# afiaka87/clip-guided-diffusion

Hardware: AMD Instinct MI355X
Metric: diffusion steps/sec (UNet+CLIP+grad) at 256x256 cutn=16 (higher is better)
Workload: dtype bf16x3 (split-bf16 MFMA, fp32 accumulate, fp32 storage); 1 GPU; BASELINE configs[1]: 256x256 class-cond UNet (554M), respace 250, cutn 16, batch 1/GPU, CLIP ViT-B/32, cgs 1000 tv 150 range 50, randomize_class, p_sample; global_batch=1, world_size_checked=1, collectives=none (single process)

## Files before the change

### clip-guided-diffusion_amd/csrc/capi.hip

```cpp
#include "../../include/cgd_mi355x.h"
#include "common.h"
#include "guidance.h"
#include "kernels.h"
#include "mfma_stage.h"
#include "net.h"

#define S(stream) ((hipStream_t)(stream))

extern "C" {

const char* cgd_version(void) { return "cgd_mi355x 0.1 (gfx950)"; }

int cgd_ctx_create(cgd_ctx** out, int device) {
  if (!out) return -3;
  cgd_ctx* ctx = new cgd_ctx();
  ctx->device = device;
  int prev = -1;
  (void)hipGetDevice(&prev);
  if (hipSetDevice(device) != hipSuccess) {
    delete ctx;
    return -1;
  }
  struct Restore {
    int d;
// ... 609 lines not shown
  return cgd_launch_conv_in(ctx, x, w, bias, y, Bn, H, W, Cin, Cout, S(stream));
}
int cgd_op_sr_stem(cgd_ctx* ctx, const float* x, const float* low, int B_low, int h, int w, const float* wpacked, const float* bias, float* y,
                   int ldy, int B, int H, int W, int Cout, void* stream) {
  CGD_NEED_CTX(ctx);
  return cgd_launch_sr_stem(ctx, x, low, B_low, h, w, wpacked, bias, y, ldy, B, H, W, Cout, S(stream));
}
int cgd_op_conv_thin_out(cgd_ctx* ctx, const float* x, int ldx, const float* w, const float* bias, float* y, int Bn, int H, int W,
                         int Cin, int Cout, void* stream) {
  CGD_NEED_CTX(ctx);
  return cgd_launch_conv_thin_out(ctx, x, ldx, w, bias, y, Bn, H, W, Cin, Cout, S(stream));
}
int64_t cgd_op_gn_scratch_floats(int B, int HW, int C) { return (int64_t)cgd_gn_scratch_floats(B, HW, C); }
int cgd_op_gn_fwd(cgd_ctx* ctx, const float* x, int ldx, float* y, int ldy, int B, int HW, int C, const float* gamma, const float* beta,
                  const float* film, int act, float eps, float* scratch, void* stream) {
  CGD_NEED_CTX(ctx);
  return cgd_launch_gn_fwd(ctx, x, ldx, y, ldy, B, HW, C, gamma, beta, film, 2 * C, act, eps, scratch, S(stream));
}
int cgd_op_gn_bwd(cgd_ctx* ctx, const float* x, int ldx, const float* dz, int lddz, float* dx, int lddx, const float* add, int ldadd,
                  int B, int HW, int C, int act, float* scratch, void* stream) {
  CGD_NEED_CTX(ctx);
  return cgd_launch_gn_bwd(ctx, x, ldx, dz, lddz, dx, lddx, add, ldadd, B, HW, C, act, scratch, S(stream));
}
int cgd_op_ln_fwd(cgd_ctx* ctx, const float* x, float* y, int rows, int C, const float* gamma, const float* beta, float eps, float* stats,
                  void* stream) {
  CGD_NEED_CTX(ctx);
  return cgd_launch_ln_fwd(ctx, x, C, y, C, rows, C, gamma, beta, eps, stats, S(stream));
}
int cgd_op_ln_bwd(cgd_ctx* ctx, const float* x, const float* dy, float* dx, int rows, int C, const float* gamma, const float* stats,
                  void* stream) {
  CGD_NEED_CTX(ctx);
  return cgd_launch_ln_bwd(ctx, x, C, dy, C, dx, C, nullptr, 0, rows, C, gamma, stats, S(stream));
}
int cgd_op_pool2x2(cgd_ctx* ctx, const float* in, float* out, int B, int Ho, int Wo, int C, float scale, void* stream) {
  CGD_NEED_CTX(ctx);
  return cgd_launch_pool2x2(ctx, in, C, out, C, nullptr, 0, B, Ho, Wo, C, scale, S(stream));
}
int cgd_op_upsample2x(cgd_ctx* ctx, const float* in, float* out, int B, int Ho, int Wo, int C, float scale, void* stream) {
  CGD_NEED_CTX(ctx);
  return cgd_launch_upsample2x(ctx, in, C, out, C, nullptr, 0, B, Ho, Wo, C, scale, S(stream));
}
int cgd_op_act(cgd_ctx* ctx, const float* x, const float* dy, float* out, int64_t n, int act, void* stream) {
  CGD_NEED_CTX(ctx);
  if (dy) return cgd_launch_act_bwd(ctx, x, dy, out, n, act, S(stream));
  return cgd_launch_act_fwd(ctx, x, out, n, act, S(stream));
}
// ... 41 lines not shown
```

### clip-guided-diffusion_amd/csrc/common.h

```cpp
#pragma once
#include <hip/hip_runtime.h>
#include <stdint.h>
#include <stdio.h>
#include <atomic>
#include <string>
#include <utility>
#include <vector>

inline std::atomic<unsigned long long> g_cgd_launches{0}, g_cgd_reduces{0};
#define CGD_LAUNCH(...)                                          \
  do {                                                           \
    g_cgd_launches.fetch_add(1, std::memory_order_relaxed);      \
    hipLaunchKernelGGL(__VA_ARGS__);                             \
  } while (0)

enum { CGD_PREC_F32 = 0, CGD_PREC_BF16X3 = 1, CGD_PREC_BF16 = 2 };

enum { CGD_PROF_GEMM = 0, CGD_PROF_HCONV = 1, CGD_PROF_GN = 2, CGD_PROF_WCONV = 3, CGD_PROF_KCONV = 4, CGD_PROF_WCONV_GNB = 5, CGD_PROF_KINDS = 6 };

struct ProfRec {
  hipEvent_t a = nullptr, b = nullptr;
  double flops = 0.0;
  int kind = 0;
  bool live = false;
};

struct SplitSrc {
  const float* ws = nullptr;
  const float* bias = nullptr;
  const float* R = nullptr;
  long stride = 0;
  int n = 0;
  int N = 0, ldr = 0;
  float alpha = 1.f;
};
struct PendingReduce {
  bool valid = false;
  SplitSrc src;
  float* C = nullptr;
  int ldc = 0, M = 0;
  hipStream_t stream = nullptr;
};

struct ChanStatsEntry {
  const float* C = nullptr;
  int ldc = 0, N = 0;
  long M = 0;
  float* buf = nullptr;
  size_t cap = 0;
  hipStream_t stream = nullptr;
  unsigned long long serial = 0;
  int kind = 0;
  int cnt = 128;
};
struct ChanSrc {
  const float* p0 = nullptr;
  const float* p1 = nullptr;
// ... 34 lines not shown
  int attn_x3 = 1;
  int attn_flash = 3;
  int fuse_act = 1;
  int fuse_gn_skip_m = 0;
  int fuse_gn_max_m = 1 << 30, fuse_gn_min_m = 4096;
  int fuse_gn = 1;
  int tile_order = 0;
  int hgemm_epi = 1;
  int hgemm_kg = 1;
  int weight_nt = 0;
  int kgemm_var = 0;
  int kgemm_big_m = 0, kgemm_big_n = 0;
  int kgemm_mode = 2, kgemm_max_m = 256;
  int hgemm_tm96 = 1;
  int hgemm_var = 1;
  int hgemm_mode = 1, hgemm_min_m = 64, hgemm_min_chunks = 4;
  PendingReduce pending;
  int defer_mode = 2;
  std::vector<ChanStatsEntry> chanstats;
  std::vector<float*> chanstats_retired;
  unsigned long long stats_serial = 1;
  unsigned long long device_allocs = 0;
  unsigned long long gn_record_merges = 0;
  bool last_wconv_bstat = false;
  int gn_epi = 3;
  std::vector<std::pair<const float*, int>> attn_fwd_path;
  std::vector<FragEntry> frag_cache;
  void* frag_tmp = nullptr;
  size_t frag_tmp_bytes = 0;
  bool prof_on = false;
  std::vector<ProfRec> prof_recs;
  std::vector<hipEvent_t> prof_pool;
  double prof_ms[CGD_PROF_KINDS] = {}, prof_flops[CGD_PROF_KINDS] = {}, prof_n[CGD_PROF_KINDS] = {};
};

struct ExactScope {
  cgd_ctx* ctx;
  int saved;
  explicit ExactScope(cgd_ctx* c) : ctx(c), saved(c->precision) { c->precision = CGD_PREC_F32; }
  ~ExactScope() { ctx->precision = saved; }
};

struct DeviceScope {
  int prev = -1;
  bool switched = false;
  explicit DeviceScope(const cgd_ctx* c) {
// ... 144 lines not shown
```

### clip-guided-diffusion_amd/csrc/kernels.h

```cpp
#pragma once
#include "common.h"

size_t cgd_gn_scratch_floats(int B, int HW, int C);
int cgd_launch_gn_fwd(cgd_ctx* ctx, const float* x, int ldx, float* y, int ldy, int B, int HW, int C, const float* gamma,
                      const float* beta, const float* film, int ldfilm, int act, float eps, float* scratch, hipStream_t s);
const float* cgd_gn_ab(const float* scratch, int B, int HW, int C);
const float* cgd_gn_coef(const float* scratch, int B, int HW, int C);
size_t cgd_gn_stats_offset(int B, int HW, int C);
int cgd_launch_gn_bwd(cgd_ctx* ctx, const float* x, int ldx, const float* dz, int lddz, float* dx, int lddx, const float* add,
                      int ldadd, int B, int HW, int C, int act, float* scratch, hipStream_t s, const float* add2 = nullptr,
                      int ldadd2 = 0);
int cgd_launch_gn_bwd_skip_gemm(cgd_ctx* ctx, GemmParams sk, const float* x, int ldx, const float* dz, int lddz, const float* add2, int ldadd2,
                                int B, int HW, int C, float* scratch, hipStream_t s, bool* done);
int cgd_launch_ln_fwd(cgd_ctx* ctx, const float* x, int ldx, float* y, int ldy, int rows, int C, const float* gamma,
                      const float* beta, float eps, float* stats, hipStream_t s);
int cgd_launch_ln_bwd(cgd_ctx* ctx, const float* x, int ldx, const float* dy, int lddy, float* dx, int lddx, const float* add,
                      int ldadd, int rows, int C, const float* gamma, const float* stats, hipStream_t s);

int cgd_launch_pool2x2(cgd_ctx* ctx, const float* in, int ldi, float* out, int ldo, const float* add, int ldadd, int B, int Ho,
                       int Wo, int C, float scale, hipStream_t s);
int cgd_launch_resample2x_pair(cgd_ctx* ctx, int up, const float* in0, int ldi0, float* out0, int ldo0, const float* in1, int ldi1, float* out1,
                               int ldo1, int B, int Ho, int Wo, int C, float scale, hipStream_t s);
int cgd_launch_upsample2x(cgd_ctx* ctx, const float* in, int ldi, float* out, int ldo, const float* add, int ldadd, int B, int Ho,
                          int Wo, int C, float scale, hipStream_t s);
int cgd_launch_copy2d(cgd_ctx* ctx, const float* a, int lda, const float* b, int ldb, float* out, int ldo, long rows, int C,
                      hipStream_t s);
int cgd_launch_concat2(cgd_ctx* ctx, const float* a, int lda, int Ca, const float* b, int ldb, int Cb, float* out, int ldo, long rows,
                       hipStream_t s);
int cgd_launch_act_fwd(cgd_ctx* ctx, const float* x, float* y, long n, int act, hipStream_t s);
int cgd_launch_act_bwd(cgd_ctx* ctx, const float* x, const float* dy, float* dx, long n, int act, hipStream_t s);
int cgd_launch_transpose(cgd_ctx* ctx, const float* in, int ldi, long si, float* out, int ldo, long so, int R, int Cc, int nb,
                         hipStream_t s);
int cgd_launch_timestep_embedding(cgd_ctx* ctx, const float* t, const float* freqs, float* out, int B, int dim, hipStream_t s);
int cgd_launch_embedding_add(cgd_ctx* ctx, const float* table, const int64_t* idx, float* out, int B, int dim, hipStream_t s);
// ... 112 lines not shown
```

### clip-guided-diffusion_amd/csrc/norm.hip

```cpp
#include "common.h"
#include "mfma_stage.h"
#include "kernels.h"

namespace {

constexpr int MAXJ = 4;
constexpr int GN_U = 4;

struct ColMap {
  int cq, TQ, rows, r, q0;
  bool active;
};
__device__ __forceinline__ ColMap col_map(int C) {
  ColMap m;
  m.cq = C >> 2;
  m.TQ = m.cq < 256 ? m.cq : 256;
  m.rows = 256 / m.TQ;
  m.r = threadIdx.x / m.TQ;
  m.q0 = threadIdx.x % m.TQ;
  m.active = m.r < m.rows;
  return m;
}

__device__ __forceinline__ float silu_f(float u) { return u / (1.f + __expf(-u)); }
// ... 686 lines not shown
template <int VEC>
__device__ __forceinline__ void vset(typename VecT<VEC>::T& v, int i, float x) {
  if constexpr (VEC == 1) v = x; else v[i] = x;
}

template <int VEC>
__device__ __forceinline__ typename VecT<VEC>::T split_load(const SplitSrc& s, long row, int col) {
  if constexpr (VEC == 1) {
    return split_load1(s, row, col);
  } else {
    const float4 a = split_load4<4>(s, row, col);
    return typename VecT<4>::T{a.x, a.y, a.z, a.w};
  }
}

template <int ACT, int VEC, bool CACHE>
__global__ __launch_bounds__(GS_NT) void gn_small_fwd_kernel(const float* x, float* xw, int ldx, float* __restrict__ y, int ldy, int HW,
                                                             int C, int lg, const float* __restrict__ gamma, const float* __restrict__ beta,
                                                             const float* __restrict__ film, int ldfilm, float eps,
                                                             float* __restrict__ stats, float* __restrict__ coef, const SplitSrc src) {
  typedef typename VecT<VEC>::T V;
  __shared__ float red[GS_NT / 64];
  __shared__ float ca[128], cb[128];
  const int g = blockIdx.x, b = blockIdx.y, cpg = C / 32, cq = cpg / VEC, n = HW * cpg;
  const int q = threadIdx.x & ((1 << lg) - 1), r = threadIdx.x >> lg, rows = GS_NT >> lg;
  const bool act_q = q < cq;
  const float* xg = x + (long)b * HW * ldx + g * cpg + q * VEC;
  float* xwg = xw + (long)b * HW * ldx + g * cpg + q * VEC;
  float* yg = y ? y + (long)b * HW * ldy + g * cpg + q * VEC : nullptr;
  const long row0 = (long)b * HW;
  const int col = g * cpg + q * VEC;
  float k0;
  {
    const int c1 = min(1, cpg - 1), c2 = min(2, cpg - 1), p1 = min(1, HW - 1), p2 = min(2, HW - 1);
    float ka, kb, kc;
    if (src.n) {
      ka = split_load1(src, row0, g * cpg);
      kb = split_load1(src, row0 + p1, g * cpg + c1);
      kc = split_load1(src, row0 + p2, g * cpg + c2);
    } else {
      const float* xk = x + (long)b * HW * ldx + g * cpg;
      ka = xk[0];
      kb = xk[(long)p1 * ldx + c1];
      kc = xk[(long)p2 * ldx + c2];
    }
    k0 = fmaxf(fminf(ka, kb), fminf(fmaxf(ka, kb), kc));
  }
  const long nrow = (long)gridDim.y * HW;
  const bool rsync = src.n && src.R && src.R < xw + nrow * ldx && xw < src.R + nrow * src.ldr;
  float s = 0.f, ss = 0.f;
  V vc[CACHE ? 8 : 1];
  if constexpr (CACHE) {
#pragma unroll
    for (int it = 0; it < 8; ++it) {
      const int p = r + it * rows;
      if (act_q && p < HW) vc[it] = src.n ? split_load<VEC>(src, row0 + p, col) : *(const V*)(xg + (long)p * ldx);
    }
    if (src.n) {
      const bool late = rsync && r < 3 && q * VEC < 3;
#pragma unroll
      for (int it = 0; it < 8; ++it) {
        const int p = r + it * rows;
        if (act_q && p < HW && !(it == 0 && late)) *(V*)(xwg + (long)p * ldx) = vc[it];
      }
      if (rsync) {
        __syncthreads();
        if (late && act_q && r < HW) *(V*)(xwg + (long)r * ldx) = vc[0];
      }
    }
#pragma unroll
    for (int it = 0; it < 8; ++it) {
      if (act_q && r + it * rows < HW) {
#pragma unroll
        for (int e = 0; e < VEC; ++e) {
          const float d = vget<VEC>(vc[it], e) - k0;
          s += d;
          ss += d * d;
        }
      }
    }
  } else {
    if (rsync) __syncthreads();
    if (act_q) {
      for (int p0 = r; p0 < HW; p0 += rows * GS_U) {
        V v[GS_U];
#pragma unroll
        for (int u = 0; u < GS_U; ++u) {
          const int p = p0 + u * rows, pc = p < HW ? p : r;
          if (src.n) {
            v[u] = split_load<VEC>(src, row0 + pc, col);
            if (p < HW) *(V*)(xwg + (long)pc * ldx) = v[u];
          } else {
            v[u] = *(const V*)(xg + (long)pc * ldx);
          }
        }
#pragma unroll
        for (int u = 0; u < GS_U; ++u) {
          if (p0 + u * rows < HW) {
#pragma unroll
            for (int e = 0; e < VEC; ++e) {
              const float d = vget<VEC>(v[u], e) - k0;
              s += d;
              ss += d * d;
            }
          }
        }
      }
    }
  }
  s = block_sum(s, red);
  ss = block_sum(ss, red);
  const float ms = s / n;
  const float mean = k0 + ms, var = fmaxf(ss / n - ms * ms, 0.f);
  const float rstd = rsqrtf(var + eps);
  if (threadIdx.x == 0) {
    stats[((long)b * 32 + g) * 2] = mean;
    stats[((long)b * 32 + g) * 2 + 1] = rstd;
  }
  if (threadIdx.x < cpg) {
    const int c = g * cpg + threadIdx.x;
    float gm = gamma[c], bt = beta[c];
    if (film) {
      const float sc = 1.f + film[(long)b * ldfilm + c], sh = film[(long)b * ldfilm + C + c];
      gm *= sc;
      bt = bt * sc + sh;
    }
    float* o = coef + ((long)b * C + c) * 4;
    o[0] = ca[threadIdx.x] = gm * rstd;
    o[1] = cb[threadIdx.x] = bt - mean * gm * rstd;
    o[2] = gm;
    o[3] = mean;
    float* ab = coef + (long)gridDim.y * C * 8 + ((long)b * C + c) * 2;
    ab[0] = o[0];
    ab[1] = o[1];
  }
  if (!y) return;
  __syncthreads();
  if (!act_q) return;
  float a[VEC], bb[VEC];
#pragma unroll
  for (int e = 0; e < VEC; ++e) {
    a[e] = ca[q * VEC + e];
    bb[e] = cb[q * VEC + e];
  }
  if constexpr (CACHE) {
#pragma unroll
    for (int it = 0; it < 8; ++it) {
      const int p = r + it * rows;
      if (p < HW) {
        V o;
#pragma unroll
        for (int e = 0; e < VEC; ++e) {
          float t = vget<VEC>(vc[it], e) * a[e] + bb[e];
          if (ACT == 1) t = silu_f(t);
          vset<VEC>(o, e, t);
        }
        *(V*)(yg + (long)p * ldy) = o;
      }
    }
    return;
  }
  for (int p0 = r; p0 < HW; p0 += rows * GS_U) {
    V v[GS_U];
#pragma unroll
    for (int u = 0; u < GS_U; ++u) {
      const int p = p0 + u * rows;
      v[u] = *(const V*)(xg + (long)(p < HW ? p : r) * ldx);
    }
#pragma unroll
    for (int u = 0; u < GS_U; ++u) {
      const int p = p0 + u * rows;
      if (p < HW) {
        V o;
#pragma unroll
        for (int e = 0; e < VEC; ++e) {
          float t = vget<VEC>(v[u], e) * a[e] + bb[e];
          if (ACT == 1) t = silu_f(t);
          vset<VEC>(o, e, t);
        }
        *(V*)(yg + (long)p * ldy) = o;
      }
    }
  }
}

template <int ACT, int VEC, bool CACHE>
__global__ __launch_bounds__(GS_NT) void gn_small_bwd_kernel(const float* __restrict__ x, int ldx, const float* dz, float* dzw, int lddz,
                                                             float* dx, int lddx, const float* add, int ldadd, const float* add2, int ldadd2,
                                                             int HW, int C, int lg, const float* __restrict__ stats,
                                                             const float* __restrict__ coef, const SplitSrc src) {
  typedef typename VecT<VEC>::T V;
  __shared__ float red[GS_NT / 64];
  const int g = blockIdx.x, b = blockIdx.y, cpg = C / 32, cq = cpg / VEC, n = HW * cpg;
  const int q = threadIdx.x & ((1 << lg) - 1), r = threadIdx.x >> lg, rows = GS_NT >> lg;
  const bool act_q = q < cq;
  const int qc = act_q ? q : 0;
  const float* xg = x + (long)b * HW * ldx + g * cpg + qc * VEC;
  const float* dg = dz + (long)b * HW * lddz + g * cpg + qc * VEC;
  float* dwg = dzw + (long)b * HW * lddz + g * cpg + qc * VEC;
  const long row0 = (long)b * HW;
  const int col = g * cpg + qc * VEC;
  float* og = dx + (long)b * HW * lddx + g * cpg + qc * VEC;
  const float* ag = add ? add + (long)b * HW * ldadd + g * cpg + qc * VEC : nullptr;
  const float* ag2 = add2 ? add2 + (long)b * HW * ldadd2 + g * cpg + qc * VEC : nullptr;
  const float mean = stats[((long)b * 32 + g) * 2], rstd = stats[((long)b * 32 + g) * 2 + 1];
  float a[VEC], bb[VEC], gc[VEC];
#pragma unroll
  for (int e = 0; e < VEC; ++e) {
    const float* o = coef + ((long)b * C + g * cpg + qc * VEC + e) * 4;
    a[e] = o[0];
    bb[e] = o[1];
    gc[e] = o[2];
  }
  float p1 = 0.f, p2 = 0.f;
  V xc[CACHE ? 4 : 1], dc[CACHE ? 4 : 1];
  if constexpr (CACHE) {
#pragma unroll
// ... 1 lines not shown
      const int p = r + it * rows;
      if (act_q && p < HW) {
        xc[it] = *(const V*)(xg + (long)p * ldx);
        dc[it] = src.n ? split_load<VEC>(src, row0 + p, col) : *(const V*)(dg + (long)p * lddz);
      }
    }
#pragma unroll
    for (int it = 0; it < 4; ++it) {
      if (act_q && r + it * rows < HW) {
#pragma unroll
        for (int e = 0; e < VEC; ++e) {
          const float xe = vget<VEC>(xc[it], e);
          float du = vget<VEC>(dc[it], e);
          if (ACT == 1) du *= dsilu_f(xe * a[e] + bb[e]);
          du *= gc[e];
          vset<VEC>(dc[it], e, du);
          p1 += du;
          p2 += du * (xe - mean);
        }
      }
    }
  } else
  if (act_q) {
    for (int p0 = r; p0 < HW; p0 += rows * GS_U) {
      V xv[GS_U], dv[GS_U];
#pragma unroll
      for (int u = 0; u < GS_U; ++u) {
        const int p = p0 + u * rows, pc = p < HW ? p : r;
        xv[u] = *(const V*)(xg + (long)pc * ldx);
        if (src.n) {
          dv[u] = split_load<VEC>(src, row0 + pc, col);
          if (p < HW) *(V*)(dwg + (long)pc * lddz) = dv[u];
        } else {
          dv[u] = *(const V*)(dg + (long)pc * lddz);
        }
      }
#pragma unroll
      for (int u = 0; u < GS_U; ++u) {
        if (p0 + u * rows < HW) {
#pragma unroll
          for (int e = 0; e < VEC; ++e) {
            const float xe = vget<VEC>(xv[u], e);
            float du = vget<VEC>(dv[u], e);
            if (ACT == 1) du *= dsilu_f(xe * a[e] + bb[e]);
            du *= gc[e];
            p1 += du;
            p2 += du * (xe - mean);
          }
        }
      }
    }
  }
  p1 = block_sum(p1, red);
  p2 = block_sum(p2, red);
  if (!act_q) return;
  const float a2 = rstd * rstd * rstd * p2 / n, a3 = rstd * p1 / n;
  if constexpr (CACHE) {
    V av[4];
#pragma unroll
    for (int it = 0; it < 4; ++it) {
      const int p = r + it * rows;
      if (ag && p < HW) av[it] = *(const V*)(ag + (long)p * ldadd);
      if (ag2 && p < HW) {
        const V a2 = *(const V*)(ag2 + (long)p * ldadd2);
        if (ag) av[it] += a2; else av[it] = a2;
      }
    }
#pragma unroll
    for (int it = 0; it < 4; ++it) {
      const int p = r + it * rows;
      if (p < HW) {
        V o;
#pragma unroll
        for (int e = 0; e < VEC; ++e) {
          float t = vget<VEC>(dc[it], e) * rstd - (vget<VEC>(xc[it], e) - mean) * a2 - a3;
          if (ag || ag2) t += vget<VEC>(av[it], e);
          vset<VEC>(o, e, t);
        }
        *(V*)(og + (long)p * lddx) = o;
      }
    }
    return;
  }
  for (int p0 = r; p0 < HW; p0 += rows * GS_U) {
    V xv[GS_U], dv[GS_U], av[GS_U];
#pragma unroll
    for (int u = 0; u < GS_U; ++u) {
      const int p = p0 + u * rows, pc = p < HW ? p : r;
      xv[u] = *(const V*)(xg + (long)pc * ldx);
      dv[u] = *(const V*)(dg + (long)pc * lddz);
      if (ag) av[u] = *(const V*)(ag + (long)pc * ldadd);
      if (ag2) {
        const V a2 = *(const V*)(ag2 + (long)pc * ldadd2);
        if (ag) av[u] += a2; else av[u] = a2;
      }
    }
#pragma unroll
    for (int u = 0; u < GS_U; ++u) {
      const int p = p0 + u * rows;
      if (p < HW) {
        V o;
#pragma unroll
        for (int e = 0; e < VEC; ++e) {
          const float xe = vget<VEC>(xv[u], e);
          float du = vget<VEC>(dv[u], e);
          if (ACT == 1) du *= dsilu_f(xe * a[e] + bb[e]);
          float t = du * gc[e] * rstd - (xe - mean) * a2 - a3;
          if (ag || ag2) t += vget<VEC>(av[u], e);
          vset<VEC>(o, e, t);
        }
        *(V*)(og + (long)p * lddx) = o;
      }
    }
  }
}

template <int ACT>
void launch_gn_small_fwd(const float* x, int ldx, float* y, int ldy, int B, int HW, int C, const float* gamma, const float* beta,
                         const float* film, int ldfilm, float eps, float* stats, float* coef, hipStream_t s, const SplitSrc& src) {
  const int cpg = C / 32;
  const bool v4 = !(cpg & 3) && !(ldx & 3) && !(ldy & 3) && !(((uintptr_t)x | (uintptr_t)y) & 15) && !(src.n && ((src.N | src.ldr) & 3));
  const int cq = v4 ? cpg / 4 : cpg;
  int lg = 0;
  while ((1 << lg) < cq) ++lg;
  const bool cache = (long)HW <= 8L * (GS_NT >> lg) && !getenv("CGD_GN_NOCACHE");
#define GN_SF(V_, C_) CGD_LAUNCH((gn_small_fwd_kernel<ACT, V_, C_>), dim3(32, B), dim3(GS_NT), 0, s, x, (float*)x, ldx, y, ldy, HW, C, lg, gamma, beta, film, ldfilm, eps, stats, coef, src)
  if (v4) {
    if (cache) GN_SF(4, true); else GN_SF(4, false);
  } else {
    if (cache) GN_SF(1, true); else GN_SF(1, false);
  }
#undef GN_SF
}

template <int ACT>
void launch_gn_small_bwd(const float* x, int ldx, const float* dz, int lddz, float* dx, int lddx, const float* add, int ldadd,
                         const float* add2, int ldadd2, int B, int HW, int C, const float* stats, const float* coef, hipStream_t s,
                         const SplitSrc& src) {
  const int cpg = C / 32;
  const bool v4 = !(cpg & 3) && !(ldx & 3) && !(lddz & 3) && !(lddx & 3) && !(ldadd & 3) && !(ldadd2 & 3) &&
                  !(((uintptr_t)x | (uintptr_t)dz | (uintptr_t)dx | (uintptr_t)add | (uintptr_t)add2) & 15) && !(src.n && ((src.N | src.ldr) & 3));
  const int cq = v4 ? cpg / 4 : cpg;
  int lg = 0;
  while ((1 << lg) < cq) ++lg;
  const bool cache = (long)HW <= 4L * (GS_NT >> lg) && !getenv("CGD_GN_NOCACHE");
#define GN_SB(V_, C_) CGD_LAUNCH((gn_small_bwd_kernel<ACT, V_, C_>), dim3(32, B), dim3(GS_NT), 0, s, x, ldx, dz, (float*)dz, lddz, dx, lddx, add, ldadd, add2, ldadd2, HW, C, lg, stats, coef, src)
  if (v4) {
    if (cache) GN_SB(4, true); else GN_SB(4, false);
  } else {
    if (cache) GN_SB(1, true); else GN_SB(1, false);
  }
#undef GN_SB
}

static int gn_small_hw() {
  static int v = -1;
  if (v < 0) {
    const char* e = getenv("CGD_GN_SMALL_HW");
    v = e ? atoi(e) : 1024;
  }
  return v;
}
#define GN_SMALL_HW gn_small_hw()

int pick_chunk(int HW, int B) {
  int chunk = HW * B / 512;
  if (chunk < 8) chunk = 8;
  if (chunk > 256) chunk = 256;
  if ((HW + chunk - 1) / chunk > 2048) chunk = (HW + 2047) / 2048;
// ... 55 lines not shown
  ChanSrc cs;
  const bool epi = !src.n && HW > GN_SMALL_HW && !(HW & 127) && (ctx->gn_epi & 1) && cgd_chanstats_find(ctx, x, ldx, (long)B * HW, C, s, &cs);
  if (y_written) cgd_chanstats_invalidate(ctx, y_written, (long)B * HW, ldy_written, C);
  ProfRec pr;
  CGD_TRY(cgd_prof_begin(ctx, &pr, CGD_PROF_GN, ((y ? 8.0 : 4.0) + (src.n ? 4.0 * src.n : 0.0)) * B * HW * C, s));
  if (epi) {
    ++ctx->gn_record_merges;
    int lg = 0;
    while ((1 << lg) < C / 32) ++lg;
    CGD_LAUNCH(gn_stats_final_ch_kernel, dim3(32, B), dim3(256), 0, s, cs, HW, C / 32, lg, eps, stats, gamma, beta, film, ldfilm, coef);
    if (y) {
      if (act)
        CGD_LAUNCH((gn_apply_kernel<1>), dim3(nchunk, B), dim3(256), 0, s, x, ldx, y, ldy, HW, C, chunk, coef);
      else
        CGD_LAUNCH((gn_apply_kernel<0>), dim3(nchunk, B), dim3(256), 0, s, x, ldx, y, ldy, HW, C, chunk, coef);
    }
    CGD_TRY(cgd_prof_stamp(ctx, &pr, s));
    cgd_prof_push(ctx, &pr);
    CGD_HIP(ctx, hipGetLastError());
    return 0;
  }
  if (HW <= GN_SMALL_HW) {
    if (act)
      launch_gn_small_fwd<1>(x, ldx, y, ldy, B, HW, C, gamma, beta, film, ldfilm, eps, stats, coef, s, src);
    else
      launch_gn_small_fwd<0>(x, ldx, y, ldy, B, HW, C, gamma, beta, film, ldfilm, eps, stats, coef, s, src);
    CGD_TRY(cgd_prof_stamp(ctx, &pr, s));
    cgd_prof_push(ctx, &pr);
    CGD_HIP(ctx, hipGetLastError());
    return 0;
  }
  CGD_LAUNCH(gn_stats_partial_kernel, dim3(nchunk, B), dim3(256), 0, s, x, (float*)x, ldx, HW, C, chunk, part, src);
  CGD_LAUNCH(gn_stats_final_kernel, dim3(32, B), dim3(256), 0, s, part, nchunk, HW, chunk, C / 32, eps, stats, gamma, beta, film,
                     ldfilm, coef);
  if (y) {
    if (act)
      CGD_LAUNCH((gn_apply_kernel<1>), dim3(nchunk, B), dim3(256), 0, s, x, ldx, y, ldy, HW, C, chunk, coef);
    else
      CGD_LAUNCH((gn_apply_kernel<0>), dim3(nchunk, B), dim3(256), 0, s, x, ldx, y, ldy, HW, C, chunk, coef);
  }
  CGD_TRY(cgd_prof_stamp(ctx, &pr, s));
  cgd_prof_push(ctx, &pr);
  CGD_HIP(ctx, hipGetLastError());
  return 0;
}

int cgd_launch_gn_bwd(cgd_ctx* ctx, const float* x, int ldx, const float* dz, int lddz, float* dx, int lddx, const float* add,
                      int ldadd, int B, int HW, int C, int act, float* scratch, hipStream_t s, const float* add2, int ldadd2) {
  if (C % 32 || C > 4096) CGD_FAIL(ctx, "groupnorm backward: C must be a multiple of 32 and <= 4096");
  if (HW > GN_SMALL_HW && (((ldx | lddz | lddx | (add ? ldadd : 0) | (add2 ? ldadd2 : 0)) & 3) ||
                           (((uintptr_t)x | (uintptr_t)dz | (uintptr_t)dx | (uintptr_t)add | (uintptr_t)add2) & 15)))
    CGD_FAIL(ctx, "groupnorm backward: above the single-launch size, row strides must be multiples of 4 and x / dz / dx / add 16-byte aligned");
  int chunk, nchunk;
  float *part, *stats, *coef, *bcoef;
  gn_layout(scratch, B, HW, C, &chunk, &nchunk, &part, &stats, &coef, &bcoef);
  SplitSrc src;
  if (!((HW > GN_SMALL_HW || ctx->defer_mode >= 2) && cgd_take_pending(ctx, dz, (long)B * HW, C, lddz, s, &src))) CGD_TRY(cgd_flush_pending(ctx, s));
  if (src.n && (((src.N | src.ldr) & 3) || ((uintptr_t)src.ws & 15) || ((uintptr_t)src.R & 15) || ((uintptr_t)src.bias & 15)) && HW > GN_SMALL_HW) {
    ctx->pending.valid = true; ctx->pending.src = src; ctx->pending.C = (float*)dz; ctx->pending.ldc = lddz; ctx->pending.M = B * HW; ctx->pending.stream = s;
    CGD_TRY(cgd_flush_pending(ctx, s));
    src = SplitSrc();
  }
  ProfRec pr;
  CGD_TRY(cgd_prof_begin(ctx, &pr, CGD_PROF_GN, (12.0 + (add ? 4.0 : 0.0) + (add2 ? 4.0 : 0.0) + (src.n ? 4.0 * src.n : 0.0)) * B * HW * C, s));
  if (HW <= GN_SMALL_HW) {
    if (act)
      launch_gn_small_bwd<1>(x, ldx, dz, lddz, dx, lddx, add, ldadd, add2, ldadd2, B, HW, C, stats, coef, s, src);
    else
      launch_gn_small_bwd<0>(x, ldx, dz, lddz, dx, lddx, add, ldadd, add2, ldadd2, B, HW, C, stats, coef, s, src);
    CGD_TRY(cgd_prof_stamp(ctx, &pr, s));
    cgd_prof_push(ctx, &pr);
    CGD_HIP(ctx, hipGetLastError());
    cgd_chanstats_invalidate(ctx, dx, (long)B * HW, lddx, C);
    return 0;
  }
  ChanSrc cs;
  const bool merged = !src.n && !(HW & 127) && (ctx->gn_epi & 2) && cgd_chanstats_find(ctx, dz, lddz, (long)B * HW, C, s, &cs, 1) && cs.n0 == C;
  cgd_chanstats_invalidate(ctx, dx, (long)B * HW, lddx, C);
  if (merged) {
    ++ctx->gn_record_merges;
    int lg = 0;
    while ((1 << lg) < C / 32) ++lg;
    CGD_LAUNCH(gn_bwd_coef_ch_kernel, dim3(32, B), dim3(256), 0, s, cs.p0, HW / cs.c0, lg, stats, coef, C, HW, bcoef);
  } else {
    if (act) {
      CGD_LAUNCH((gn_bwd_partial_kernel<1>), dim3(nchunk, B), dim3(256), 0, s, x, ldx, dz, (float*)dz, lddz, HW, C, chunk, coef, part, src);
    } else {
      CGD_LAUNCH((gn_bwd_partial_kernel<0>), dim3(nchunk, B), dim3(256), 0, s, x, ldx, dz, (float*)dz, lddz, HW, C, chunk, coef, part, src);
    }
    CGD_LAUNCH(gn_bwd_coef_kernel, dim3(32, B), dim3(256), 0, s, part, nchunk, stats, coef, C, HW, bcoef);
  }
  if (act) {
// ... 140 lines not shown
  for (float* p : ctx->chanstats_retired) (void)hipFree(p);
  ctx->chanstats.clear();
  ctx->chanstats_retired.clear();
}

void cgd_chanstats_invalidate(cgd_ctx* ctx, const float* C, long rows, int ld, int cols) {
  if (!C || rows <= 0 || ctx->chanstats.empty()) return;
  const float* end = C + (rows - 1) * (long)ld + cols;
  for (ChanStatsEntry& q : ctx->chanstats) {
    if (q.serial != ctx->stats_serial) continue;
    const float* qend = q.C + (q.M - 1) * (long)q.ldc + q.N;
    if (!(q.C < end && C < qend)) continue;
    if (q.ldc == ld && ld > 0) {
      long d = (q.C - C) % ld;
      if (d < 0) d += ld;
      const bool cols_apart = (d >= cols && d + q.N <= ld) ;
      if (cols_apart) continue;
    }
    q.serial = 0;
  }
}

bool cgd_gn_merges_records(int HW) { return HW > GN_SMALL_HW && !(HW & 127); }
```

### clip-guided-diffusion_amd/lib.py

```python
import ctypes as C
import os
import weakref

_HERE = os.path.dirname(os.path.abspath(__file__))
LIB_PATH = os.environ.get("CGD_LIB_PATH") or os.path.join(_HERE, "libcgd_mi355x.so")

F32P = C.POINTER(C.c_float)
vp = C.c_void_p
i32 = C.c_int
i64 = C.c_int64
f32 = C.c_float


class UNetConfig(C.Structure):
    _fields_ = [
        ("image_size", i32), ("model_channels", i32), ("num_res_blocks", i32), ("n_mult", i32),
        ("channel_mult", f32 * 8), ("n_att", i32), ("attention_ds", i32 * 8), ("num_classes", i32),
        ("num_heads", i32), ("num_head_channels", i32), ("use_new_attention_order", i32),
        ("in_channels", i32), ("out_channels", i32),
        ("classic_resample", i32), ("additive_emb", i32),
    ]


class ClassifierConfig(C.Structure):
# ... 199 lines not shown
    "cgd_op_conv3x3_s2": (i32, [vp, vp, i32, vp, vp, vp, i32, i32, i32, i32, i32, i32, vp]),
    "cgd_op_conv3x3_s2_dgrad": (i32, [vp, vp, i32, vp, vp, i32, vp, i32, i32, i32, i32, i32, i32, vp]),
    "cgd_op_conv3x3_s2_accepts": (i32, [i32] * 9),
    "cgd_op_conv3x3_s2_packed": (i32, [vp, vp, i32, vp, vp, vp, i32, i32, i32, i32, i32, i32, vp]),
    "cgd_op_conv3x3_s2_dgrad_packed": (i32, [vp, vp, i32, vp, vp, i32, vp, i32, i32, i32, i32, i32, i32, vp]),
    "cgd_op_conv3x3": (i32, [vp, vp, i32, vp, vp, vp, i32, vp, vp, i32, i32, i32, i32, i32, i32, i32, i32, i32, vp]),
    "cgd_op_conv3x3_ex": (i32, [vp, vp, i32, vp, vp, vp, i32, vp, vp, i32, vp, i32, i32, i32, i32, i32, i32, i32, i32, i32, i32, vp, i32, vp, vp]),
    "cgd_op_pack_conv3x3_wino": (i32, [vp, vp, vp, i32, i32, i32, vp]),
    "cgd_op_conv3x3_wino": (i32, [vp, vp, i32, vp, vp, i32, vp, vp, i32, vp, i32, i32, i32, i32, i32, i32, vp]),
    "cgd_set_wino": (i32, [vp, i32, i32]),
    "cgd_op_conv3x3_wino_ex": (i32, [vp, vp, i32, vp, vp, i32, vp, vp, i32, vp, i32, i32, i32, i32, i32, i32, i32, vp, i32, vp, vp]),
    "cgd_op_new_pass": (i32, [vp]),
    "cgd_op_gn_record_merges": (i64, [vp]),
    "cgd_op_gn_records": (i32, [vp, vp, i32, i64, i32, i32, vp, i64, C.POINTER(i32), vp]),
    "cgd_op_gn_stats_offset": (i64, [i32, i32, i32]),
    "cgd_op_wconv_schedule": (i32, [i32, i32, C.POINTER(i32)]),
    "cgd_op_mfma_peak": (i32, [vp, i32, C.POINTER(C.c_double), vp]),
    "cgd_op_conv_in": (i32, [vp, vp, vp, vp, vp, i32, i32, i32, i32, i32, vp]),
    "cgd_op_conv_thin_out": (i32, [vp, vp, i32, vp, vp, vp, i32, i32, i32, i32, i32, vp]),
    "cgd_op_sr_stem": (i32, [vp, vp, vp, i32, i32, i32, vp, vp, vp, i32, i32, i32, i32, i32, vp]),
    "cgd_op_gn_scratch_floats": (i64, [i32, i32, i32]),
    "cgd_op_gn_fwd": (i32, [vp, vp, i32, vp, i32, i32, i32, i32, vp, vp, vp, i32, f32, vp, vp]),
    "cgd_op_gn_bwd": (i32, [vp, vp, i32, vp, i32, vp, i32, vp, i32, i32, i32, i32, i32, vp, vp]),
    "cgd_op_ln_fwd": (i32, [vp, vp, vp, i32, i32, vp, vp, f32, vp, vp]),
    "cgd_op_ln_bwd": (i32, [vp, vp, vp, vp, i32, i32, vp, vp, vp]),
    "cgd_op_pool2x2": (i32, [vp, vp, vp, i32, i32, i32, i32, f32, vp]),
    "cgd_op_upsample2x": (i32, [vp, vp, vp, i32, i32, i32, i32, f32, vp]),
    "cgd_op_act": (i32, [vp, vp, vp, vp, i64, i32, vp]),
    "cgd_op_attn_buf_floats": (i64, [i32, i32, i32, i32, i32]),
    "cgd_op_attn_buf_floats_ctx": (i64, [vp, i32, i32, i32, i32, i32, i32, i32]),
    "cgd_op_attn_fwd": (i32, [vp, vp, vp, i32, i32, i32, i32, i32, C.POINTER(vp), vp]),
    "cgd_op_attn_bwd": (i32, [vp, vp, vp, vp, i32, i32, i32, i32, i32, C.POINTER(vp), vp]),
    "cgd_op_attn_fwd_causal": (i32, [vp, vp, vp, i32, i32, i32, i32, C.POINTER(vp), vp]),
    "cgd_op_attn_plan": (i32, [i32, i32, i32, i32, i32, i32, C.POINTER(i32)]),
}

EXPORTED_SYMBOLS = tuple(_SIGS)

_lib = None


def load():
    global _lib
    if _lib is None:
        if not os.path.isfile(LIB_PATH):
            raise RuntimeError(
# ... 85 lines not shown
```

### include/cgd_mi355x.h

```cpp
#ifndef CGD_MI355X_H
#define CGD_MI355X_H
#include <stdint.h>

#ifdef __cplusplus
extern "C" {
#endif

typedef struct cgd_ctx cgd_ctx;
typedef struct cgd_unet cgd_unet;
typedef struct cgd_vit cgd_vit;

enum { CGD_F32 = 0, CGD_BF16X3 = 1, CGD_BF16 = 2 };

int cgd_ctx_create(cgd_ctx** out, int device);
void cgd_ctx_destroy(cgd_ctx* ctx);
const char* cgd_last_error(cgd_ctx* ctx);
int cgd_set_precision(cgd_ctx* ctx, int mode);
int cgd_get_precision(cgd_ctx* ctx);
int64_t cgd_ctx_device_allocs(cgd_ctx* ctx);
const char* cgd_version(void);
int cgd_set_tiles(cgd_ctx* ctx, int large_tile, int small_tile);
int cgd_set_hgemm(cgd_ctx* ctx, int mode, int min_m, int min_chunks);
int cgd_profile(cgd_ctx* ctx, int enable);
int cgd_profile_read(cgd_ctx* ctx, double* out18);
// ... 321 lines not shown
                            int ldadd, int B, int H, int W, int Cin, int Cout, void* stream);
int cgd_op_conv3x3_s2_accepts(int dgrad, int ld_in, int ld_out, int ldadd, int B, int H, int W, int Cin, int Cout);
int cgd_op_conv3x3_s2_packed(cgd_ctx* ctx, const float* x_nhwc, int ldx, const float* w_fwd, const float* bias, float* y_nhwc, int ldy, int B,
                             int H, int W, int Cin, int Cout, void* stream);
int cgd_op_conv3x3_s2_dgrad_packed(cgd_ctx* ctx, const float* dy_nhwc, int lddy, const float* w_dgrad, float* dx_nhwc, int lddx,
                                   const float* add, int ldadd, int B, int H, int W, int Cin, int Cout, void* stream);
int cgd_op_new_pass(cgd_ctx* ctx);
int64_t cgd_op_gn_record_merges(cgd_ctx* ctx);
int cgd_op_gn_records(cgd_ctx* ctx, const float* y, int ldy, int64_t rows, int C, int kind, float* out, int64_t cap, int* pixels, void* stream);
int64_t cgd_op_gn_stats_offset(int B, int HW, int C);
int cgd_op_wconv_schedule(int nb, int q, int* out7);
int cgd_op_mfma_peak(cgd_ctx* ctx, int iters, double* flop_out, void* stream);
int cgd_op_conv_in(cgd_ctx* ctx, const float* x_nchw, const float* w, const float* bias, float* y_nhwc, int Bn, int H, int W, int Cin,
                   int Cout, void* stream);
int cgd_op_conv_thin_out(cgd_ctx* ctx, const float* x_nhwc, int ldx, const float* w, const float* bias, float* y_nchw, int Bn, int H,
                         int W, int Cin, int Cout, void* stream);
int cgd_op_sr_stem(cgd_ctx* ctx, const float* x, const float* low, int B_low, int h, int w, const float* wpacked, const float* bias, float* y,
                   int ldy, int B, int H, int W, int Cout, void* stream);
int64_t cgd_op_gn_scratch_floats(int B, int HW, int C);
int cgd_op_gn_fwd(cgd_ctx* ctx, const float* x, int ldx, float* y, int ldy, int B, int HW, int C, const float* gamma,
                  const float* beta, const float* film, int act, float eps, float* scratch, void* stream);
int cgd_op_gn_bwd(cgd_ctx* ctx, const float* x, int ldx, const float* dz, int lddz, float* dx, int lddx, const float* add, int ldadd,
                  int B, int HW, int C, int act, float* scratch, void* stream);
int cgd_op_ln_fwd(cgd_ctx* ctx, const float* x, float* y, int rows, int C, const float* gamma, const float* beta, float eps,
                  float* stats, void* stream);
int cgd_op_ln_bwd(cgd_ctx* ctx, const float* x, const float* dy, float* dx, int rows, int C, const float* gamma, const float* stats,
                  void* stream);
int cgd_op_pool2x2(cgd_ctx* ctx, const float* in, float* out, int B, int Ho, int Wo, int C, float scale, void* stream);
int cgd_op_upsample2x(cgd_ctx* ctx, const float* in, float* out, int B, int Ho, int Wo, int C, float scale, void* stream);
int cgd_op_act(cgd_ctx* ctx, const float* x, const float* dy, float* out, int64_t n, int act, void* stream);
int64_t cgd_op_attn_buf_floats(int nb, int heads, int T, int d, int which);
int64_t cgd_op_attn_buf_floats_ctx(cgd_ctx* ctx, int nb, int heads, int T, int d, int legacy, int causal, int which);
int cgd_op_attn_fwd(cgd_ctx* ctx, const float* qkv, float* out, int nb, int heads, int T, int d, int legacy, float* bufs[5],
                    void* stream);
int cgd_op_attn_bwd(cgd_ctx* ctx, const float* qkv, const float* dout, float* dqkv, int nb, int heads, int T, int d, int legacy,
                    float* bufs[5], void* stream);
int cgd_op_attn_fwd_causal(cgd_ctx* ctx, const float* qkv, float* out, int nb, int heads, int T, int d, float* bufs[5], void* stream);
int cgd_op_attn_plan(int T, int d, int ldq, int ldo, int precision, int attn_flash, int* out2);

#ifdef __cplusplus
}
#endif
#endif
```

Measured before the change: 58.20 diffusion steps/sec.

## Split small-HW GroupNorm work across partner blocks per group

The small-spatial GroupNorm forward and backward kernels can now launch k partner workgroups per (group, batch) instead of one. Each partner recomputes the full group statistics redundantly, but only writes its own share of rows or unrolled vectors. A launcher policy picks k from the per-group slab size and the number of streams, and falls back to one block when input and output buffers alias. This aims to fill more of the GPU for batch-1 low-resolution layers, which otherwise launch only 32 blocks. The cost is duplicated reads and reductions per partner.

```diff
diff --git a/clip-guided-diffusion_amd/csrc/capi.hip b/clip-guided-diffusion_amd/csrc/capi.hip
--- a/clip-guided-diffusion_amd/csrc/capi.hip
+++ b/clip-guided-diffusion_amd/csrc/capi.hip
@@ -655,6 +655,28 @@
   CGD_NEED_CTX(ctx);
   return cgd_launch_gn_bwd(ctx, x, ldx, dz, lddz, dx, lddx, add, ldadd, B, HW, C, act, scratch, S(stream));
 }
+int cgd_op_gn_bwd2(cgd_ctx* ctx, const float* x, int ldx, const float* dz, int lddz, float* dx, int lddx, const float* add, int ldadd,
+                   const float* add2, int ldadd2, int B, int HW, int C, int act, float* scratch, void* stream) {
+  CGD_NEED_CTX(ctx);
+  return cgd_launch_gn_bwd(ctx, x, ldx, dz, lddz, dx, lddx, add, ldadd, B, HW, C, act, scratch, S(stream), add2, ldadd2);
+}
+int cgd_set_gn_partners(cgd_ctx* ctx, int k) {
+  CGD_NEED_CTX(ctx);
+  if (k != 0 && k != 1 && k != 2 && k != 4 && k != 8) CGD_FAIL(ctx, "cgd_set_gn_partners: k must be 0 (the launcher's policy), 1, 2, 4 or 8");
+  ctx->gn_partners = k;
+  return 0;
+}
+int cgd_op_gn_partners(cgd_ctx* ctx, int bwd, const float* x, int ldx, const float* dz, int lddz, const float* out, int ldout, const float* R,
+                       int ldr, int slices, int nadd, int B, int HW, int C, int force) {
+  if (!ctx && force < 0) return -3;
+  if ((force > 2 && force != 4 && force != 8) || HW < 1 || HW > 1024 || C < 32 || C % 32 || slices < 0 || nadd < 0 || nadd > 2 || !x || (bwd && !dz))
+    return -1;
+  SplitSrc src;
+  if (slices) {
+    src.ws = ctx ? ctx->ws : nullptr; src.n = slices; src.N = C; src.stride = (long)B * HW * C; src.R = R; src.ldr = ldr;
+  }
+  return cgd_gn_small_partners(force < 0 ? ctx->gn_partners : force, bwd, x, ldx, dz, lddz, out, ldout, nadd, src, B, HW, C);
+}
 int cgd_op_ln_fwd(cgd_ctx* ctx, const float* x, float* y, int rows, int C, const float* gamma, const float* beta, float eps, float* stats,
                   void* stream) {
   CGD_NEED_CTX(ctx);
diff --git a/clip-guided-diffusion_amd/csrc/common.h b/clip-guided-diffusion_amd/csrc/common.h
--- a/clip-guided-diffusion_amd/csrc/common.h
+++ b/clip-guided-diffusion_amd/csrc/common.h
@@ -33,6 +33,16 @@
   int n = 0;
   int N = 0, ldr = 0;
   float alpha = 1.f;
+};
+struct GnShare {
+  int g, part, km, blk0, blk1;
+  __device__ __forceinline__ GnShare(int HW, int block_rows) {
+    const int k = gridDim.x >> 5, nblk = (HW + block_rows - 1) / block_rows;
+    g = blockIdx.x & 31, part = blockIdx.x >> 5, km = k - 1;
+    blk0 = part * nblk / k, blk1 = (part + 1) * nblk / k;
+  }
+  __device__ __forceinline__ bool vec(int it) const { return (it & km) == part; }
+  __device__ __forceinline__ bool block(int blk) const { return blk >= blk0 && blk < blk1; }
 };
 struct PendingReduce {
   bool valid = false;
@@ -113,6 +123,7 @@
   unsigned long long stats_serial = 1;
   unsigned long long device_allocs = 0;
   unsigned long long gn_record_merges = 0;
+  int gn_partners = 0;
   bool last_wconv_bstat = false;
   int gn_epi = 3;
   std::vector<std::pair<const float*, int>> attn_fwd_path;
diff --git a/clip-guided-diffusion_amd/csrc/kernels.h b/clip-guided-diffusion_amd/csrc/kernels.h
--- a/clip-guided-diffusion_amd/csrc/kernels.h
+++ b/clip-guided-diffusion_amd/csrc/kernels.h
@@ -10,6 +10,8 @@
 int cgd_launch_gn_bwd(cgd_ctx* ctx, const float* x, int ldx, const float* dz, int lddz, float* dx, int lddx, const float* add,
                       int ldadd, int B, int HW, int C, int act, float* scratch, hipStream_t s, const float* add2 = nullptr,
                       int ldadd2 = 0);
+int cgd_gn_small_partners(int force, int bwd, const float* x, int ldx, const float* dz, int lddz, const float* out, int ldout, int nadd,
+                          const SplitSrc& src, int B, int HW, int C);
 int cgd_launch_gn_bwd_skip_gemm(cgd_ctx* ctx, GemmParams sk, const float* x, int ldx, const float* dz, int lddz, const float* add2, int ldadd2,
                                 int B, int HW, int C, float* scratch, hipStream_t s, bool* done);
 int cgd_launch_ln_fwd(cgd_ctx* ctx, const float* x, int ldx, float* y, int ldy, int rows, int C, const float* gamma,
diff --git a/clip-guided-diffusion_amd/csrc/norm.hip b/clip-guided-diffusion_amd/csrc/norm.hip
--- a/clip-guided-diffusion_amd/csrc/norm.hip
+++ b/clip-guided-diffusion_amd/csrc/norm.hip
@@ -732,8 +732,8 @@
   typedef typename VecT<VEC>::T V;
   __shared__ float red[GS_NT / 64];
   __shared__ float ca[128], cb[128];
-  const int g = blockIdx.x, b = blockIdx.y, cpg = C / 32, cq = cpg / VEC, n = HW * cpg;
-  const int q = threadIdx.x & ((1 << lg) - 1), r = threadIdx.x >> lg, rows = GS_NT >> lg;
+  const GnShare sh(HW, (GS_NT >> lg) * GS_U);
+  const int g = sh.g, b = blockIdx.y, cpg = C / 32, cq = cpg / VEC, n = HW * cpg, q = threadIdx.x & ((1 << lg) - 1), r = threadIdx.x >> lg, rows = GS_NT >> lg;
   const bool act_q = q < cq;
   const float* xg = x + (long)b * HW * ldx + g * cpg + q * VEC;
   float* xwg = xw + (long)b * HW * ldx + g * cpg + q * VEC;
@@ -771,11 +771,11 @@
 #pragma unroll
       for (int it = 0; it < 8; ++it) {
         const int p = r + it * rows;
-        if (act_q && p < HW && !(it == 0 && late)) *(V*)(xwg + (long)p * ldx) = vc[it];
+        if (act_q && p < HW && sh.vec(it) && !(it == 0 && late)) *(V*)(xwg + (long)p * ldx) = vc[it];
       }
       if (rsync) {
         __syncthreads();
-        if (late && act_q && r < HW) *(V*)(xwg + (long)r * ldx) = vc[0];
+        if (late && act_q && r < HW && sh.vec(0)) *(V*)(xwg + (long)r * ldx) = vc[0];
       }
     }
 #pragma unroll
@@ -792,14 +792,14 @@
   } else {
     if (rsync) __syncthreads();
     if (act_q) {
-      for (int p0 = r; p0 < HW; p0 += rows * GS_U) {
+      for (int p0 = r, blk = 0; p0 < HW; p0 += rows * GS_U, ++blk) {
         V v[GS_U];
 #pragma unroll
         for (int u = 0; u < GS_U; ++u) {
           const int p = p0 + u * rows, pc = p < HW ? p : r;
           if (src.n) {
             v[u] = split_load<VEC>(src, row0 + pc, col);
-            if (p < HW) *(V*)(xwg + (long)pc * ldx) = v[u];
+            if (p < HW && sh.block(blk)) *(V*)(xwg + (long)pc * ldx) = v[u];
           } else {
             v[u] = *(const V*)(xg + (long)pc * ldx);
           }
@@ -823,7 +823,7 @@
   const float ms = s / n;
   const float mean = k0 + ms, var = fmaxf(ss / n - ms * ms, 0.f);
   const float rstd = rsqrtf(var + eps);
-  if (threadIdx.x == 0) {
+  if (threadIdx.x == 0 && sh.part == 0) {
     stats[((long)b * 32 + g) * 2] = mean;
     stats[((long)b * 32 + g) * 2 + 1] = rstd;
   }
@@ -836,13 +836,13 @@
       bt = bt * sc + sh;
     }
     float* o = coef + ((long)b * C + c) * 4;
-    o[0] = ca[threadIdx.x] = gm * rstd;
-    o[1] = cb[threadIdx.x] = bt - mean * gm * rstd;
-    o[2] = gm;
-    o[3] = mean;
+    const float fa = ca[threadIdx.x] = gm * rstd, fb = cb[threadIdx.x] = bt - mean * gm * rstd;
     float* ab = coef + (long)gridDim.y * C * 8 + ((long)b * C + c) * 2;
-    ab[0] = o[0];
-    ab[1] = o[1];
+    if (sh.part == 0) {
+      o[0] = ab[0] = fa;
+      o[1] = ab[1] = fb;
+      o[2] = gm, o[3] = mean;
+    }
   }
   if (!y) return;
   __syncthreads();
@@ -857,7 +857,7 @@
 #pragma unroll
     for (int it = 0; it < 8; ++it) {
       const int p = r + it * rows;
-      if (p < HW) {
+      if (p < HW && sh.vec(it)) {
         V o;
 #pragma unroll
         for (int e = 0; e < VEC; ++e) {
@@ -870,7 +870,7 @@
     }
     return;
   }
-  for (int p0 = r; p0 < HW; p0 += rows * GS_U) {
+  for (int p0 = r + sh.blk0 * rows * GS_U; p0 < HW && p0 < sh.blk1 * rows * GS_U; p0 += rows * GS_U) {
     V v[GS_U];
 #pragma unroll
     for (int u = 0; u < GS_U; ++u) {
@@ -901,8 +901,8 @@
                                                              const float* __restrict__ coef, const SplitSrc src) {
   typedef typename VecT<VEC>::T V;
   __shared__ float red[GS_NT / 64];
-  const int g = blockIdx.x, b = blockIdx.y, cpg = C / 32, cq = cpg / VEC, n = HW * cpg;
-  const int q = threadIdx.x & ((1 << lg) - 1), r = threadIdx.x >> lg, rows = GS_NT >> lg;
+  const GnShare sh(HW, (GS_NT >> lg) * GS_U);
+  const int g = sh.g, b = blockIdx.y, cpg = C / 32, cq = cpg / VEC, n = HW * cpg, q = threadIdx.x & ((1 << lg) - 1), r = threadIdx.x >> lg, rows = GS_NT >> lg;
   const bool act_q = q < cq;
   const int qc = act_q ? q : 0;
   const float* xg = x + (long)b * HW * ldx + g * cpg + qc * VEC;
@@ -950,7 +950,7 @@
     }
   } else
   if (act_q) {
-    for (int p0 = r; p0 < HW; p0 += rows * GS_U) {
+    for (int p0 = r, blk = 0; p0 < HW; p0 += rows * GS_U, ++blk) {
       V xv[GS_U], dv[GS_U];
 #pragma unroll
       for (int u = 0; u < GS_U; ++u) {
@@ -958,7 +958,7 @@
         xv[u] = *(const V*)(xg + (long)pc * ldx);
         if (src.n) {
           dv[u] = split_load<VEC>(src, row0 + pc, col);
-          if (p < HW) *(V*)(dwg + (long)pc * lddz) = dv[u];
+          if (p < HW && sh.block(blk)) *(V*)(dwg + (long)pc * lddz) = dv[u];
         } else {
           dv[u] = *(const V*)(dg + (long)pc * lddz);
         }
@@ -988,8 +988,8 @@
 #pragma unroll
     for (int it = 0; it < 4; ++it) {
       const int p = r + it * rows;
-      if (ag && p < HW) av[it] = *(const V*)(ag + (long)p * ldadd);
-      if (ag2 && p < HW) {
+      if (ag && p < HW && sh.vec(it)) av[it] = *(const V*)(ag + (long)p * ldadd);
+      if (ag2 && p < HW && sh.vec(it)) {
         const V a2 = *(const V*)(ag2 + (long)p * ldadd2);
         if (ag) av[it] += a2; else av[it] = a2;
       }
@@ -997,7 +997,7 @@
 #pragma unroll
     for (int it = 0; it < 4; ++it) {
       const int p = r + it * rows;
-      if (p < HW) {
+      if (p < HW && sh.vec(it)) {
         V o;
 #pragma unroll
         for (int e = 0; e < VEC; ++e) {
@@ -1010,7 +1010,7 @@
     }
     return;
   }
-  for (int p0 = r; p0 < HW; p0 += rows * GS_U) {
+  for (int p0 = r + sh.blk0 * rows * GS_U; p0 < HW && p0 < sh.blk1 * rows * GS_U; p0 += rows * GS_U) {
     V xv[GS_U], dv[GS_U], av[GS_U];
 #pragma unroll
     for (int u = 0; u < GS_U; ++u) {
@@ -1045,14 +1045,14 @@
 
 template <int ACT>
 void launch_gn_small_fwd(const float* x, int ldx, float* y, int ldy, int B, int HW, int C, const float* gamma, const float* beta,
-                         const float* film, int ldfilm, float eps, float* stats, float* coef, hipStream_t s, const SplitSrc& src) {
+                         const float* film, int ldfilm, float eps, float* stats, float* coef, hipStream_t s, const SplitSrc& src, int force) {
   const int cpg = C / 32;
   const bool v4 = !(cpg & 3) && !(ldx & 3) && !(ldy & 3) && !(((uintptr_t)x | (uintptr_t)y) & 15) && !(src.n && ((src.N | src.ldr) & 3));
   const int cq = v4 ? cpg / 4 : cpg;
   int lg = 0;
   while ((1 << lg) < cq) ++lg;
   const bool cache = (long)HW <= 8L * (GS_NT >> lg) && !getenv("CGD_GN_NOCACHE");
-#define GN_SF(V_, C_) CGD_LAUNCH((gn_small_fwd_kernel<ACT, V_, C_>), dim3(32, B), dim3(GS_NT), 0, s, x, (float*)x, ldx, y, ldy, HW, C, lg, gamma, beta, film, ldfilm, eps, stats, coef, src)
+#define GN_SF(V_, C_) CGD_LAUNCH((gn_small_fwd_kernel<ACT, V_, C_>), dim3(32 * cgd_gn_small_partners(force, 0, x, ldx, nullptr, 0, y, ldy, 0, src, B, HW, C), B), dim3(GS_NT), 0, s, x, (float*)x, ldx, y, ldy, HW, C, lg, gamma, beta, film, ldfilm, eps, stats, coef, src)
   if (v4) {
     if (cache) GN_SF(4, true); else GN_SF(4, false);
   } else {
@@ -1064,15 +1064,15 @@
 template <int ACT>
 void launch_gn_small_bwd(const float* x, int ldx, const float* dz, int lddz, float* dx, int lddx, const float* add, int ldadd,
                          const float* add2, int ldadd2, int B, int HW, int C, const float* stats, const float* coef, hipStream_t s,
-                         const SplitSrc& src) {
-  const int cpg = C / 32;
+                         const SplitSrc& src, int force) {
+  const int cpg = C / 32, nadd = (add != nullptr) + (add2 != nullptr);
   const bool v4 = !(cpg & 3) && !(ldx & 3) && !(lddz & 3) && !(lddx & 3) && !(ldadd & 3) && !(ldadd2 & 3) &&
                   !(((uintptr_t)x | (uintptr_t)dz | (uintptr_t)dx | (uintptr_t)add | (uintptr_t)add2) & 15) && !(src.n && ((src.N | src.ldr) & 3));
   const int cq = v4 ? cpg / 4 : cpg;
   int lg = 0;
   while ((1 << lg) < cq) ++lg;
   const bool cache = (long)HW <= 4L * (GS_NT >> lg) && !getenv("CGD_GN_NOCACHE");
-#define GN_SB(V_, C_) CGD_LAUNCH((gn_small_bwd_kernel<ACT, V_, C_>), dim3(32, B), dim3(GS_NT), 0, s, x, ldx, dz, (float*)dz, lddz, dx, lddx, add, ldadd, add2, ldadd2, HW, C, lg, stats, coef, src)
+#define GN_SB(V_, C_) CGD_LAUNCH((gn_small_bwd_kernel<ACT, V_, C_>), dim3(32 * cgd_gn_small_partners(force, 1, x, ldx, dz, lddz, dx, lddx, nadd, src, B, HW, C), B), dim3(GS_NT), 0, s, x, ldx, dz, (float*)dz, lddz, dx, lddx, add, ldadd, add2, ldadd2, HW, C, lg, stats, coef, src)
   if (v4) {
     if (cache) GN_SB(4, true); else GN_SB(4, false);
   } else {
@@ -1174,9 +1174,9 @@
   }
   if (HW <= GN_SMALL_HW) {
     if (act)
-      launch_gn_small_fwd<1>(x, ldx, y, ldy, B, HW, C, gamma, beta, film, ldfilm, eps, stats, coef, s, src);
+      launch_gn_small_fwd<1>(x, ldx, y, ldy, B, HW, C, gamma, beta, film, ldfilm, eps, stats, coef, s, src, ctx->gn_partners);
     else
-      launch_gn_small_fwd<0>(x, ldx, y, ldy, B, HW, C, gamma, beta, film, ldfilm, eps, stats, coef, s, src);
+      launch_gn_small_fwd<0>(x, ldx, y, ldy, B, HW, C, gamma, beta, film, ldfilm, eps, stats, coef, s, src, ctx->gn_partners);
     CGD_TRY(cgd_prof_stamp(ctx, &pr, s));
     cgd_prof_push(ctx, &pr);
     CGD_HIP(ctx, hipGetLastError());
@@ -1217,9 +1217,9 @@
   CGD_TRY(cgd_prof_begin(ctx, &pr, CGD_PROF_GN, (12.0 + (add ? 4.0 : 0.0) + (add2 ? 4.0 : 0.0) + (src.n ? 4.0 * src.n : 0.0)) * B * HW * C, s));
   if (HW <= GN_SMALL_HW) {
     if (act)
-      launch_gn_small_bwd<1>(x, ldx, dz, lddz, dx, lddx, add, ldadd, add2, ldadd2, B, HW, C, stats, coef, s, src);
+      launch_gn_small_bwd<1>(x, ldx, dz, lddz, dx, lddx, add, ldadd, add2, ldadd2, B, HW, C, stats, coef, s, src, ctx->gn_partners);
     else
-      launch_gn_small_bwd<0>(x, ldx, dz, lddz, dx, lddx, add, ldadd, add2, ldadd2, B, HW, C, stats, coef, s, src);
+      launch_gn_small_bwd<0>(x, ldx, dz, lddz, dx, lddx, add, ldadd, add2, ldadd2, B, HW, C, stats, coef, s, src, ctx->gn_partners);
     CGD_TRY(cgd_prof_stamp(ctx, &pr, s));
     cgd_prof_push(ctx, &pr);
     CGD_HIP(ctx, hipGetLastError());
@@ -1406,3 +1406,44 @@
 }
 
 bool cgd_gn_merges_records(int HW) { return HW > GN_SMALL_HW && !(HW & 127); }
+
+static int gn_partner_policy(int bwd, long slab, int streams) {
+  if (slab >= 96 * 1024) return 8;
+  if (slab >= 48 * 1024 && bwd && streams >= 2) return 4;
+  return 1;
+}
+
+int cgd_gn_small_partners(int force, int bwd, const float* x, int ldx, const float* dz, int lddz, const float* out, int ldout, int nadd,
+                          const SplitSrc& src, int B, int HW, int C) {
+  if (!out) return 1;
+  const long rows = (long)B * HW;
+  struct Span { const float* p; long n; };
+  Span rd[4], wr[2];
+  int nr = 0, nw = 0;
+  wr[nw++] = {out, rows * ldout};
+  const float* sliced = bwd ? dz : x;
+  const int ldsl = bwd ? lddz : ldx;
+  if (bwd) rd[nr++] = {x, rows * ldx};
+  if (src.n) {
+    wr[nw++] = {sliced, rows * ldsl};
+    if (src.ws) rd[nr++] = {src.ws, (long)(src.n - 1) * src.stride + rows * src.N};
+    if (src.R) rd[nr++] = {src.R, rows * src.ldr};
+  } else {
+    rd[nr++] = {sliced, rows * ldsl};
+  }
+  for (int i = 0; i < nw; ++i)
+    for (int j = 0; j < nr; ++j)
+      if (wr[i].p < rd[j].p + rd[j].n && rd[j].p < wr[i].p + wr[i].n) return 1;
+  if (force) return force;
+  const int cpg = C / 32;
+  int lg = 0;
+  while ((1 << lg) < ((cpg & 3) ? cpg : cpg / 4)) ++lg;
+  const int rows_wg = GS_NT >> lg;
+  const bool cache = (long)HW <= (bwd ? 4L : 8L) * rows_wg;
+  const int shares = cache ? cdiv(HW, rows_wg) : cdiv(HW, rows_wg * GS_U);
+  const long slab = (long)HW * cpg * 4;
+  const int streams = 1 + (bwd ? nadd : 0) + (src.n && !(bwd && cache) ? 1 : 0);
+  int k = gn_partner_policy(bwd, slab, streams);
+  while (k > 1 && k > shares) k >>= 1;
+  return k;
+}
diff --git a/clip-guided-diffusion_amd/lib.py b/clip-guided-diffusion_amd/lib.py
--- a/clip-guided-diffusion_amd/lib.py
+++ b/clip-guided-diffusion_amd/lib.py
@@ -245,6 +245,9 @@
     "cgd_op_gn_scratch_floats": (i64, [i32, i32, i32]),
     "cgd_op_gn_fwd": (i32, [vp, vp, i32, vp, i32, i32, i32, i32, vp, vp, vp, i32, f32, vp, vp]),
     "cgd_op_gn_bwd": (i32, [vp, vp, i32, vp, i32, vp, i32, vp, i32, i32, i32, i32, i32, vp, vp]),
+    "cgd_op_gn_bwd2": (i32, [vp, vp, i32, vp, i32, vp, i32, vp, i32, vp, i32, i32, i32, i32, i32, vp, vp]),
+    "cgd_set_gn_partners": (i32, [vp, i32]),
+    "cgd_op_gn_partners": (i32, [vp, i32, vp, i32, vp, i32, vp, i32, vp, i32, i32, i32, i32, i32, i32, i32]),
     "cgd_op_ln_fwd": (i32, [vp, vp, vp, i32, i32, vp, vp, f32, vp, vp]),
     "cgd_op_ln_bwd": (i32, [vp, vp, vp, vp, i32, i32, vp, vp, vp]),
     "cgd_op_pool2x2": (i32, [vp, vp, vp, i32, i32, i32, i32, f32, vp]),
diff --git a/include/cgd_mi355x.h b/include/cgd_mi355x.h
--- a/include/cgd_mi355x.h
+++ b/include/cgd_mi355x.h
@@ -367,6 +367,11 @@
                   const float* beta, const float* film, int act, float eps, float* scratch, void* stream);
 int cgd_op_gn_bwd(cgd_ctx* ctx, const float* x, int ldx, const float* dz, int lddz, float* dx, int lddx, const float* add, int ldadd,
                   int B, int HW, int C, int act, float* scratch, void* stream);
+int cgd_op_gn_bwd2(cgd_ctx* ctx, const float* x, int ldx, const float* dz, int lddz, float* dx, int lddx, const float* add, int ldadd,
+                   const float* add2, int ldadd2, int B, int HW, int C, int act, float* scratch, void* stream);
+int cgd_set_gn_partners(cgd_ctx* ctx, int k);
+int cgd_op_gn_partners(cgd_ctx* ctx, int bwd, const float* x, int ldx, const float* dz, int lddz, const float* out, int ldout, const float* R,
+                       int ldr, int slices, int nadd, int B, int HW, int C, int force);
 int cgd_op_ln_fwd(cgd_ctx* ctx, const float* x, float* y, int rows, int C, const float* gamma, const float* beta, float eps,
                   float* stats, void* stream);
 int cgd_op_ln_bwd(cgd_ctx* ctx, const float* x, const float* dy, float* dx, int rows, int C, const float* gamma, const float* stats,
```

Measured after the change: 58.46 diffusion steps/sec (median of 6 runs). About the same (+0.4%).
